# Lweihan/LDiffusion

Measured on AMD Instinct MI355X. Metric: patches/sec (512x512, 5 denoise steps), higher is better.
Workload: dtype f16 (fp32 accumulate)

## Files before the change

ldiffusion_amd/csrc/common.h:

```cpp
#pragma once
#include <hip/hip_runtime.h>
#include <stdint.h>
#include <stdio.h>
#include <string>
#include <vector>

typedef _Float16 f16;
typedef _Float16 f16x2 __attribute__((ext_vector_type(2)));
typedef _Float16 f16x4 __attribute__((ext_vector_type(4)));
typedef _Float16 f16x8 __attribute__((ext_vector_type(8)));
typedef float f32x4 __attribute__((ext_vector_type(4)));
typedef short s16x4 __attribute__((ext_vector_type(4)));

#include "../../include/ldiff.h"
void ldiff_set_error(const char* fmt, ...);

struct LdiffError {
  int code;
};
#define LDIFF_CHECK(cond, code, ...)     \
  do {                                   \
    if (!(cond)) {                       \
      ldiff_set_error(__VA_ARGS__);      \
      throw LdiffError{code};            \
// ... 56 lines not shown
  int silu_out = 0, cond_force = 0;
  int lrelu_in = 0, tconv = 0;
  int seg_conv = 0;
  int relu_out = 0, cls_force = 0;
  int* nonfinite = nullptr;
  int act_out = 0;
  int plan_B = 0, plan_M = 0;
};
inline ConvParams nominal_launch(const ConvParams& p) {
  ConvParams q = p;
  if (p.plan_B > 0) { q.B = p.plan_B; q.M = p.plan_M; }
  return q;
}
constexpr int LO8_SHIFT = 15;
void launch_lo8_weights(const f16* w, void* wd, int* scale_out, int Nrows, int taps, int Cin, hipStream_t s);
enum class ConvKernel { COND , TCONV , SEGCONV , CLSCONV , C3_NARROW, C3_NARROW_FOLD, C3_DATAFLOW, C3_PINGPONG, C3_HALO, GEMM_DF, GEMM_DMA, IGEMM, NONE  };
enum class ConvWeights { PLAIN, FRAG, FRAG_PAR, FRAG_SC, GEMM_FRAG };
struct ConvAsk {
  int splitk = 0;
  bool stats = false;
  bool fold_gn = false;
};
struct ConvPlan {
  ConvKernel kernel = ConvKernel::NONE;
  ConvWeights weights = ConvWeights::PLAIN;
  bool parity = false;
  bool fold_gn = false;
  int bm = 0, bn = 0;
};
ConvPlan plan_conv(ConvParams& p, const ConvAsk& ask);
size_t parity_weights_bytes(const ConvParams& p);
void pack_parity_weights(const ConvParams& p, f16* dst, hipStream_t s);
size_t packed_weights_bytes(ConvWeights layout, const ConvParams& p);
void pack_weights(ConvWeights layout, const ConvParams& p, const f16* sc_w, f16* dst, hipStream_t s);
void pack_shortcut_bias(const ConvParams& p, const float* sc_bias, float* dst, hipStream_t s);
bool conv_lo8_enabled();
void launch_igemm(const ConvParams& p, const ConvPlan& pl, hipStream_t s);
bool cond_conv_selected(const ConvParams& p);
void launch_cond_conv(const ConvParams& p, hipStream_t s);
void launch_tconv2x2(const ConvParams& p, hipStream_t s);
bool segconv_selected(const ConvParams& p);
int segconv_stats_blocks(const ConvParams& p);
void launch_segconv(const ConvParams& p, hipStream_t s);
void launch_in_finalize(const float* part, int R, const f16* x_or_null, int ldx, int B, int HW, int C, float eps, const float* gamma, const float* beta, float* scale, float* shift,
                        int ld_ss, int ss_off, int ident , hipStream_t s, int* nonfinite);
void launch_nhwc_f32_to_nchw(const float* x, void* y, int B, int C, int H, int W, int ldx, int out_f16, hipStream_t s);
bool cls_conv_selected(const ConvParams& p);
void launch_cls_conv(const ConvParams& p, hipStream_t s);
void launch_maxpool3x3s2(const f16* x, f16* y, int B, int H, int W, int C, hipStream_t s);
void launch_crop_resize_norm(const uint8_t* rgb, int H, int W, const int* boxes, int n, const uint8_t* lut, int S, const double* mean3, const double* std3, f16* out, hipStream_t s);
void launch_cls_head(const f16* x, int B, int HW, int A, int ldx, const float* w, const float* bias, int C, float* logits, int* labels_or_null, hipStream_t s);
void launch_scale_f16(const f16* x, f16* y, float a, long long n, hipStream_t s);
bool conv3x3_eligible(const ConvParams& p);
void launch_splitk_reduce(const ConvParams& p, hipStream_t s);
void launch_make_parity_weights(const f16* w, f16* w_par, int Nrows, int Cin, hipStream_t s);
void launch_conv3x3(const ConvParams& p, int bm, int bn, hipStream_t s);
bool conv3x3n_selected(const ConvParams& p);
bool conv3x3nt_selected(const ConvParams& p);
void launch_conv3x3n(const ConvParams& p, bool fold, hipStream_t s);
bool conv3x3p_selected(const ConvParams& p);
bool conv3x3d_selected(const ConvParams& p);
int conv3x3d_stats_blocks(const ConvParams& p);
size_t conv3x3d_frag_bytes(const ConvParams& p);
void launch_pack_frag_weights(const f16* w, f16* wf, int N, int Cin, hipStream_t s);
void launch_pack_frag_weights_par(const f16* wpar, f16* wf, int N, int Nrows, int Cin, hipStream_t s);
void launch_pack_frag_weights_sc(const f16* wsc, f16* wf, int N, int Cin, int Cs, int ld_wsc, hipStream_t s);
void launch_add_vectors(const float* a, const float* b, float* out, int n, hipStream_t s);
void launch_conv3x3d(const ConvParams& p, hipStream_t s);
int conv3x3p_stats_blocks(const ConvParams& p);
void launch_conv3x3p(const ConvParams& p, hipStream_t s);
bool lngemm_eligible(int C, int N, int ldx, int x_lo, int ldy, bool geglu);
void launch_lngemm_tile_weights(const f16* w, f16* wt, int N, int C, hipStream_t s);
void launch_lngemm(const f16* x, int ldx, int x_lo, int M, int C, const float* gamma, const float* beta, float eps, const f16* w_tiled, int N,
                   const float* bias, bool geglu, f16* y, int ldy, hipStream_t s, int qcols = 0, float qscale = 1.0f,
                   int plan_M = 0);
bool gemm_dma_eligible(const ConvParams& p);
bool gemm_df_selected(const ConvParams& p);
size_t gemm_df_frag_bytes(const ConvParams& p);
void launch_pack_gemm_frag(const f16* w, f16* wf, int Nrows, int K, hipStream_t s);
void launch_gemm_df(const ConvParams& p, hipStream_t s);
void launch_gemm_dma(const ConvParams& p, int bm, int bn, hipStream_t s);

struct AttnParams {
  const f16* q; int ldq;
  const f16* k; int ldk;
  const f16* v; int ldv;
  f16* o; int ldo;
  int B, heads, Lq, Lk, d;
  long long q_bstride, kv_bstride, o_bstride;
  float scale;
  int prescaled = 0;
  float rescale_log2 = 0.0f;
  int xcd_order = 0;
  int plan_B = 0;
};
void launch_attention(const AttnParams& p, hipStream_t s);
bool attention_prescale_supported(int d);

void launch_text_embed(const int* ids, const float* tok, const float* pos, f16* y, int M, int L, int H, int vocab, hipStream_t s);
bool text_attention_supported(int d, int L);
void launch_text_attention(const f16* qkv, int ld, int hidden, f16* o, int ldo, int o_lo , int B, int heads, int L, int d, float scale,
                           hipStream_t s);
void launch_text_ln(const f16* x_split, int M, int C, const float* gamma, const float* beta, float eps, void* out, int out_f16, f16* y_split, int* nonfinite, hipStream_t s);
void launch_f32_to_f16(const float* x, f16* y, long long n, hipStream_t s);

struct SrcView { const f16* p; int C, ld, lo; };
// ... 285 lines not shown
```

ldiffusion_amd/csrc/conv_route.hip:

```cpp
#include "common.h"

namespace {

long long tiles(const ConvParams& p, int bm, int bn) { return (long long)((p.M + bm - 1) / bm) * ((p.N + bn - 1) / bn); }
bool n_small(const ConvParams& p) { return p.N <= 64 || (p.N % 128 != 0 && p.N % 128 <= 64 && p.N < 512); }
int splits(long long t, int nk) { int S = (int)(512 / t); S = S > nk / 16 ? nk / 16 : S; return S > 8 ? 8 : S; }

int splitk_by_model(long long tiles, int steps, int min_steps, double partial_bytes, int s_old, int s_cap = 16) {
  auto T = [&](int S) {
    const double wgs = (double)tiles * S, per = (steps + S - 1) / S;
    return 4.0 + per * 0.95 * (wgs > 330.0 ? wgs / 330.0 : 1.0) + (S > 1 ? 4.0 + 2.0 * S * partial_bytes / 3.0e6 : 0.0);
  };
  if (s_old < 1) s_old = 1;
  int best = s_old;
  double tb = T(s_old);
  for (int S = s_old + 1; S <= s_cap && steps / S >= min_steps; ++S)
    if (T(S) < tb) { tb = T(S); best = S; }
  return tb <= 0.85 * T(s_old) ? best : s_old;
}

void c3_tile(const ConvParams& p, ConvPlan& pl) {
  pl.bm = (p.w_par ? p.Win : p.Wout) >= 16 ? 128 : 64;
  pl.bn = (p.N % 128 != 0 && p.N % 160 == 0) ? 160 : (p.N <= 32 ? 32 : (p.N <= 64 ? 64 : 128));
}
// ... 72 lines not shown
  LDIFF_CHECK(!q.act_out || !(q.relu_out || q.cls_force > 0 || q.silu_out || q.cond_force > 0 || q.tconv || q.lrelu_in || q.seg_conv > 0), LDIFF_ERR_INVALID,
              "conv: act_out cannot be combined with relu_out / cls_conv = 1 / silu_out / cond_conv = 1 / tconv / lrelu_in / seg_conv = 1 (only the LDS-DMA GEMM has that epilogue)");
  if (ask.splitk < 2 && cond_conv_selected(q)) {
    pl.kernel = ConvKernel::COND;
    p.splitk = 0;
    p.stats_R = 0;
    return pl;
  }
  LDIFF_CHECK(!q.lrelu_in || (q.gn_scale && q.gn_shift && !q.silu_in && (q.lrelu_in & ~3) == 0), LDIFF_ERR_INVALID, "conv: lrelu_in = %d needs gn_scale / gn_shift, silu_in = 0 and bits 0..1 only", q.lrelu_in);
  if (q.tconv) {
    LDIFF_CHECK(q.tconv == 1 && q.ks == 2 && q.stride == 2 && !q.ups && !q.x2 && q.C2 == 0 && q.C1 % 8 == 0 && q.Hout == 2 * q.Hin && q.Wout == 2 * q.Win && q.N == q.Nrows && q.N % 16 == 0 &&
                    q.K == q.C1 && !q.res && !q.temb && !q.out_f32 && !q.y_lo && !q.geglu && !q.silu_in && !q.silu_out && !q.out_shift && !q.xs && !q.lo8_slab0 && ask.splitk < 2 && !ask.stats &&
                    q.ldy >= q.N && q.ldy % 4 == 0 && (q.ld1 == 0 || (q.ld1 >= q.C1 && q.ld1 % 8 == 0)) && (long long)q.B * q.Hin * q.Win == q.M / 4 && q.M % 4 == 0,
                LDIFF_ERR_INVALID, "conv: tconv takes kernel = stride = 2, one source with C1 %% 8 == 0, N == Nrows, N %% 16 == 0, Hout = 2 Hin, a plain fp16 output and bias only (C1=%d N=%d Nrows=%d ks=%d stride=%d)",
                q.C1, q.N, q.Nrows, q.ks, q.stride);
    pl.kernel = ConvKernel::TCONV;
    p.splitk = 0;
    p.stats_R = 0;
    return pl;
  }
  if (ask.splitk < 2 && segconv_selected(q)) {
    pl.kernel = ConvKernel::SEGCONV;
    p.splitk = 0;
    p.stats_R = ask.stats ? segconv_stats_blocks(q) : 0;
    return pl;
  }
  if (ask.splitk < 2 && !ask.stats && cls_conv_selected(q)) {
    pl.kernel = ConvKernel::CLSCONV;
    p.splitk = 0;
    p.stats_R = 0;
    return pl;
  }
  LDIFF_CHECK(!q.relu_out && q.ks != 7, LDIFF_ERR_INVALID, "conv: a ReLU epilogue (relu_out) and 7x7 taps exist only in the classifier's conv family, which does not take this launch (Cin=%d N=%d ks=%d stride=%d pad=%d cls_conv=%d)",
              q.C1 + q.C2, q.N, q.ks, q.stride, q.pad_t, q.cls_force);
  LDIFF_CHECK(!q.silu_out, LDIFF_ERR_INVALID, "conv: a SiLU epilogue (silu_out) exists only in the conditioning-embedding kernel, which does not take this launch (Cin=%d N=%d ks=%d stride=%d)",
              q.C1 + q.C2, q.N, q.ks, q.stride);
  if (q.act_out) {
    LDIFF_CHECK((q.act_out == 1 || q.act_out == 2) && !q.geglu && !q.res && !q.out_f32 && !q.out_shift && !q.gn_scale && !q.temb && !ask.stats && ask.splitk < 2 && q.w_bstride == 0 &&
                    !q.xs && !q.lo8_slab0 && p.df_force <= 0 && gemm_dma_eligible(q),
                LDIFF_ERR_INVALID, "conv: act_out = %d (1 quick_gelu | 2 gelu) exists only in the LDS-DMA GEMM: a linear layer (ks = 1, K %% 64 == 0) with bias and an fp16 output (plain or split), no residual / "
                "fp32 output / GEGLU / statistics / range shift / split-K / gemm_df (C1=%d C2=%d N=%d ks=%d stride=%d)", q.act_out, q.C1, q.C2, q.N, q.ks, q.stride);
    pl.kernel = ConvKernel::GEMM_DMA;
    gemm_dma_tile(q, 1, pl);
    p.splitk = 0;
    p.stats_R = 0;
    return pl;
  }
  if (ask.fold_gn && q.gn_scale && !q.silu_in && !q.lrelu_in && q.ks == 1 && !q.x2 && !q.out_f32 && !q.geglu) {
    ConvParams f = q;
    f.gn_scale = nullptr; f.gn_shift = nullptr;
    f.w_bstride = (long long)q.Nrows * q.K; f.bias_bstride = q.Nrows;
    if (gemm_dma_eligible(f)) { q = f; pl.fold_gn = true; }
  }
  const bool c3 = conv3x3_eligible(q) && !(q.lrelu_in && q.ups), gemm = !c3 && !q.lrelu_in && gemm_dma_eligible(q);
  pl.parity = q.ups && c3;
  if (pl.parity) q.w_par = reinterpret_cast<const f16*>(placeholder);
  if (ask.splitk >= 2) {
    LDIFF_CHECK(ask.splitk <= (c3 ? (q.C1 + q.C2) / 64 : (q.K + 63) / 64), LDIFF_ERR_INVALID, "conv: more splits than K steps (%d)", ask.splitk);
    q.splitk = ask.splitk;
  } else if (ask.splitk == 0 && !q.out_f32) {
    q.splitk = c3 ? conv3x3_splitk_plan(q) : gemm ? gemm_dma_splitk_plan(q) : igemm_splitk_plan(q);
  }
  if (q.splitk < 2) q.splitk = 0;
  const int hw = q.Hout * q.Wout;
  const bool rows32 = q.splitk > 1 || !c3;
  q.stats = nullptr; q.stats_R = 0;
  if (ask.stats && !q.out_f32 && hw > 0 && (!rows32 || hw % 32 == 0)) {
    q.stats = placeholder;
    q.stats_R = rows32 ? hw / 32 : 0;
  }
  if (c3) {
    const bool par = pl.parity;
    const int Ht = par ? q.Hin : q.Hout, Wt = par ? q.Win : q.Wout;
    if (q.lrelu_in) {
      pl.kernel = ConvKernel::C3_HALO;
      c3_tile(q, pl);
    } else if (q.lo8_slab0) pl.kernel = q.splitk <= 1 && conv3x3p_selected(q) ? ConvKernel::C3_PINGPONG : ConvKernel::NONE;
    else if (conv3x3n_selected(q)) pl.kernel = conv3x3nt_selected(q) ? ConvKernel::C3_NARROW_FOLD : ConvKernel::C3_NARROW;
    else if (conv3x3d_selected(q)) pl.kernel = ConvKernel::C3_DATAFLOW;
    else if (conv3x3p_selected(q)) pl.kernel = ConvKernel::C3_PINGPONG;
    else {
      pl.kernel = ConvKernel::C3_HALO;
      c3_tile(q, pl);
    }
    if (q.stats && !rows32) {
      if (q.lo8_slab0 || pl.kernel == ConvKernel::C3_PINGPONG) q.stats_R = conv3x3p_stats_blocks(q);
      else if (pl.kernel == ConvKernel::C3_DATAFLOW) q.stats_R = conv3x3d_stats_blocks(q);
      else {
        const int TW = pl.bm / 8;
        q.stats_R = ((Ht + 7) / 8) * ((Wt + TW - 1) / TW) * (TW == 16 ? 1 : 2) * (par ? 4 : 1);
      }
    }
  } else if (gemm) {
    if (gemm_df_selected(q)) pl.kernel = ConvKernel::GEMM_DF;
    else {
      pl.kernel = ConvKernel::GEMM_DMA;
      gemm_dma_tile(q, q.splitk > 1 ? q.splitk : 1, pl);
    }
  } else {
    pl.kernel = ConvKernel::IGEMM;
    igemm_tile(q, q.splitk > 1 ? q.splitk : 1, pl);
  }
  if (pl.kernel == ConvKernel::C3_DATAFLOW) pl.weights = q.xs ? ConvWeights::FRAG_SC : pl.parity ? ConvWeights::FRAG_PAR : ConvWeights::FRAG;
  else if (pl.kernel == ConvKernel::GEMM_DF) pl.weights = ConvWeights::GEMM_FRAG;

  p.splitk = q.splitk;
  p.stats_R = q.stats_R;
  if (pl.fold_gn) {
    p.gn_scale = nullptr; p.gn_shift = nullptr;
    p.w_bstride = q.w_bstride; p.bias_bstride = q.bias_bstride;
  }
  return pl;
}

size_t parity_weights_bytes(const ConvParams& p) { return (size_t)4 * p.Nrows * 4 * (p.C1 + p.C2) * sizeof(f16); }
void pack_parity_weights(const ConvParams& p, f16* dst, hipStream_t s) { launch_make_parity_weights(p.w, dst, p.Nrows, p.C1 + p.C2, s); }
size_t packed_weights_bytes(ConvWeights layout, const ConvParams& p) {
  return layout == ConvWeights::PLAIN ? 0 : layout == ConvWeights::GEMM_FRAG ? gemm_df_frag_bytes(p) : conv3x3d_frag_bytes(p);
}
void pack_weights(ConvWeights layout, const ConvParams& p, const f16* sc_w, f16* dst, hipStream_t s) {
  switch (layout) {
    case ConvWeights::PLAIN: break;
    case ConvWeights::FRAG_PAR: launch_pack_frag_weights_par(p.w_par, dst, p.N, p.Nrows, p.C1, s); break;
    case ConvWeights::FRAG:
    case ConvWeights::FRAG_SC:
      launch_pack_frag_weights(p.w, dst, p.N, p.C1, s);
      if (layout == ConvWeights::FRAG_SC) launch_pack_frag_weights_sc(sc_w, dst, p.N, p.C1, p.Cs, p.Cs, s);
// ... 6 lines not shown
```

ldiffusion_amd/csrc/kernels_conv3x3.hip:

```cpp
#include "common.h"

namespace {

__device__ __forceinline__ int swz8(int row, int chunk) { return chunk ^ ((row >> 1) & 7); }

typedef __attribute__((address_space(1))) const void gptr_t;
typedef __attribute__((address_space(3))) void lptr_t;

template <int TH, int TW, int BN, bool GN, bool LR = false>
__global__ __launch_bounds__(256, 2) void conv3x3_kernel(const ConvParams p) {
  constexpr int BM = TH * TW, HWD = TW + 2, HP = (TH + 2) * (TW + 2);
  constexpr int MT = BM / 32, NT = BN / 32;
  constexpr int A_IT = (HP * 8 + 255) / 256, W_IT = BN * 8 / 256;
  static_assert(BN % 32 == 0 && (BN * 8) % 256 == 0, "BN must be a multiple of 32");
  extern __shared__ __attribute__((aligned(16))) unsigned char smem_raw[];
  uint4* sA = reinterpret_cast<uint4*>(smem_raw);
  uint4* sW = sA + 2 * HP * 8;

  const int tid = threadIdx.x, lane = tid & 63;
  const int wave = __builtin_amdgcn_readfirstlane(tid >> 6);
  const int wave_m = wave >> 1, wave_n = wave & 1;
  const int g = lane >> 4, l15 = lane & 15;
  const int Cin = p.C1 + p.C2;
  const bool par = p.w_par != nullptr;
// ... 212 lines not shown
      if (p.res) { v += up4(rr[m][a]); if (p.res_lo) v += up4(rl[m][a]); }
      if (p.out_f32) {
        *reinterpret_cast<f32x4*>(reinterpret_cast<float*>(p.y) + mrow[m] * p.ldy + n) = v;
      } else {
        const f16x4 o = cvt4(v);
        *reinterpret_cast<f16x4*>(reinterpret_cast<f16*>(p.y) + mrow[m] * p.ldy + n) = o;
        if (p.y_lo) *reinterpret_cast<f16x4*>(reinterpret_cast<f16*>(p.y) + mrow[m] * p.ldy + p.y_lo + n) = cvt4(v - up4(o));
        if (p.stats) acc[a][m] = p.y_lo ? split_stat4(v) : up4(o);
      }
    }
  }
  if (p.stats) {
    bool ok[MT];
#pragma unroll
    for (int m = 0; m < MT; ++m) ok[m] = mrow[m] >= 0;
    const long long R = p.stats_R, rblk = (((long long)q_par * tiles_y + ty) * tiles_x + tx) * 2 + wave_m;
    wave_stats_store<MT, NT>(acc, ok, 0, MT, p.stats + ((long long)b * p.N * R + rblk) * 2, R, p.N, ncol, l15);
  }
}

template <int I, int N, class F>
__device__ __forceinline__ void static_for(F&& f) {
  if constexpr (I < N) { f(std::integral_constant<int, I>{}); static_for<I + 1, N>(f); }
}
template <int OFF>
__device__ __forceinline__ void lds_read128(f16x8& d, unsigned addr) {
  asm volatile("ds_read_b128 %0, %1 offset:%2" : "=v"(d) : "v"(addr), "n"(OFF) : "memory");
}
template <int CNT>
__device__ __forceinline__ void lds_wait(f16x8& a) { asm volatile("s_waitcnt lgkmcnt(%1)" : "+v"(a) : "n"(CNT)); }
template <int CNT>
__device__ __forceinline__ void lds_wait(f16x8& a, f16x8& b, f16x8& c, f16x8& d, f16x8& e) {
  asm volatile("s_waitcnt lgkmcnt(%5)" : "+v"(a), "+v"(b), "+v"(c), "+v"(d), "+v"(e) : "n"(CNT));
}

__device__ __forceinline__ int swzx(int hx) { return (0xcb5888 >> (3 * (hx >> 1))) & 7; }

#ifdef C3W_STAMPS
__device__ unsigned long long c3w_dbg[32];
__device__ __forceinline__ unsigned long long w_stamp() {
  __builtin_amdgcn_sched_barrier(0);
  unsigned long long t = __builtin_amdgcn_s_memtime();
  asm volatile("s_waitcnt lgkmcnt(0)" ::: "memory");
  __builtin_amdgcn_sched_barrier(0);
  return t;
}
#define WSTAMP(v) const unsigned long long v = w_stamp()
#define WACC(i, expr) wdbg[i] += (expr)
#else
#define WSTAMP(v)
#define WACC(i, expr)
#endif

template <int BN, bool GN, bool LR = false>
__global__ __launch_bounds__(256, BN > 128 ? 1 : 2) void conv3x3w_kernel(const ConvParams p) {
  constexpr int TH = 8, TW = 16, BM = 128, HWD = 18, HP = 180, MT = 4, NT = BN / 32, A_IT = 6, NP = BN / 32;
  constexpr int ROWB = HWD * 128;
#ifdef C3W_RING2
  constexpr bool R3 = false;
#else
  constexpr bool R3 = BN == 160;
#endif
  constexpr int NSLOT = R3 ? 3 : 2;
  constexpr unsigned W_OFF = 2 * HP * 128, W_BYTES = BN * 128;
  constexpr unsigned DUMP = W_OFF + NSLOT * W_BYTES;
  constexpr int NF = NT + MT;
  extern __shared__ __attribute__((aligned(16))) unsigned char smem_raw[];

  const int tid = threadIdx.x, lane = tid & 63;
  const int wave = __builtin_amdgcn_readfirstlane(tid >> 6);
  const int wave_m = wave >> 1, wave_n = wave & 1;
  const int g = lane >> 4, l15 = lane & 15;
  const int Cin = p.C1 + p.C2;
  const bool par = p.w_par != nullptr;
  const int Ht = par ? p.Hin : p.Hout, Wt = par ? p.Win : p.Wout;
  const int tiles_x = (Wt + TW - 1) / TW, tiles_y = (Ht + TH - 1) / TH;
  const int ntn = (p.N + BN - 1) / BN;
  int nwg = gridDim.x, id = blockIdx.x;
  int q8 = nwg >> 3, r8 = nwg & 7, xcd = id & 7, idx = id >> 3;
  int sw = (xcd < r8 ? xcd * (q8 + 1) : r8 * (q8 + 1) + (xcd - r8) * q8) + idx;
  auto fdiv = [](int n, unsigned m) { return m ? (int)__umulhi((unsigned)n, m) : n; };
  int tm, tile_n;
  if (p.img_fast) { tile_n = fdiv(sw, p.div_tm); tm = sw - tile_n * p.tiles_m; }
  else { tm = fdiv(sw, p.div_ntn); tile_n = sw - tm * ntn; }
  const int q_par = par ? tm & 3 : 0, py = q_par >> 1, px = q_par & 1;
  tm = par ? tm >> 2 : tm;
  const int tq = fdiv(tm, p.div_tx);
  const int tx = tm - tq * tiles_x;
  const int b = fdiv(tq, p.div_ty);
  const int ty = tq - b * tiles_y;
  const int n0 = tile_n * BN, oy0 = ty * TH, ox0 = tx * TW;
  const int sh = par ? 0 : p.ups;
  const int He = p.Hin << sh, We = p.Win << sh;
  const unsigned lds0 = (unsigned)(size_t)(lptr_t*)smem_raw;
#ifdef C3W_STAMPS
  unsigned long long wdbg[32] = {0};
  WSTAMP(w_t0);
#endif

  const int kc = tid & 7;
  unsigned a_pix[A_IT], a_msk[A_IT], a_lds[A_IT];
#pragma unroll
  for (int i = 0; i < A_IT; ++i) {
    const int hp = (tid >> 3) + i * 32;
    const int hy = hp / HWD, hx = hp - hy * HWD;
    const int iy = oy0 + hy - 1, ix = ox0 + hx - 1;
    const bool inb = hp < HP && iy >= 0 && iy < He && ix >= 0 && ix < We;
    a_pix[i] = inb ? (unsigned)(((b * p.Hin + (iy >> sh)) * p.Win) + (ix >> sh)) : 0u;
    a_msk[i] = inb ? 0xffffffffu : 0u;
    a_lds[i] = hp < HP ? (unsigned)(hp * 128 + ((kc ^ swzx(hx)) << 4)) : DUMP + (unsigned)((tid - 160) * 16);
  }
  uint4 ra[A_IT];
  float4 gs0, gs1, gt0, gt1;
  float lslope = 1.0f;
  auto load_halo = [&](int c) {
    const int cb = c * 64;
    const f16* src; int cs, Cs;
    if (cb < p.C1) { src = p.x; cs = cb; Cs = p.ld1 ? p.ld1 : p.C1; } else { src = p.x2; cs = cb - p.C1; Cs = p.ld2 ? p.ld2 : p.C2; }
    if (LR) lslope = ((cb < p.C1 ? p.lrelu_in : p.lrelu_in >> 1) & 1) ? 0.01f : 1.0f;
    src += cs + kc * 8;
#pragma unroll
    for (int i = 0; i < A_IT; ++i) ra[i] = *reinterpret_cast<const uint4*>(src + (size_t)a_pix[i] * (unsigned)Cs);
    if (GN) {
      const float* sc = p.gn_scale + (long long)b * Cin + cb + kc * 8;
      const float* st = p.gn_shift + (long long)b * Cin + cb + kc * 8;
      gs0 = *reinterpret_cast<const float4*>(sc); gs1 = *reinterpret_cast<const float4*>(sc + 4);
      gt0 = *reinterpret_cast<const float4*>(st); gt1 = *reinterpret_cast<const float4*>(st + 4);
    }
  };
  const int nslab_all = Cin >> 6, S = p.splitk > 1 ? p.splitk : 1, ksplit = blockIdx.y;
  int c_begin = 0, nslab = nslab_all;
  if (S > 1) { c_begin = ksplit * nslab_all / S; nslab = (ksplit + 1) * nslab_all / S; }
  load_halo(c_begin);
  __builtin_amdgcn_sched_barrier(0);
  const bool silu = p.silu_in != 0;
  auto xform_store = [&](auto ic, unsigned bufoff) {
    constexpr int i = decltype(ic)::value;
    uint4 v = ra[i];
    if constexpr (LR) {
      v.x = in_lrelu_pair(ra[i].x, gs0.x, gt0.x, gs0.y, gt0.y, lslope); v.y = in_lrelu_pair(ra[i].y, gs0.z, gt0.z, gs0.w, gt0.w, lslope);
      v.z = in_lrelu_pair(ra[i].z, gs1.x, gt1.x, gs1.y, gt1.y, lslope); v.w = in_lrelu_pair(ra[i].w, gs1.z, gt1.z, gs1.w, gt1.w, lslope);
    } else if (GN) {
      if (silu) {
        v.x = gn_pair<true>(ra[i].x, gs0.x, gt0.x, gs0.y, gt0.y); v.y = gn_pair<true>(ra[i].y, gs0.z, gt0.z, gs0.w, gt0.w);
        v.z = gn_pair<true>(ra[i].z, gs1.x, gt1.x, gs1.y, gt1.y); v.w = gn_pair<true>(ra[i].w, gs1.z, gt1.z, gs1.w, gt1.w);
      } else {
        v.x = gn_pair<false>(ra[i].x, gs0.x, gt0.x, gs0.y, gt0.y); v.y = gn_pair<false>(ra[i].y, gs0.z, gt0.z, gs0.w, gt0.w);
        v.z = gn_pair<false>(ra[i].z, gs1.x, gt1.x, gs1.y, gt1.y); v.w = gn_pair<false>(ra[i].w, gs1.z, gt1.z, gs1.w, gt1.w);
      }
    }
    v.x &= a_msk[i]; v.y &= a_msk[i]; v.z &= a_msk[i]; v.w &= a_msk[i];
    *reinterpret_cast<uint4*>(smem_raw + bufoff + a_lds[i]) = v;
  };

  const long long Kw = (long long)(par ? 4 : 9) * Cin;
  const f16* wsrc = par ? p.w_par + (long long)q_par * p.Nrows * Kw : p.w;
  const __amdgpu_buffer_rsrc_t wrsrc = __builtin_amdgcn_make_buffer_rsrc((void*)wsrc, 0, (int)((long long)p.Nrows * Kw * 2), 0x00020000);
  int w_voff[NP];
#pragma unroll
  for (int i = 0; i < NP; ++i) {
    const int r = wave * (BN / 4) + i * 8 + (lane >> 3), pos = lane & 7;
    int n = n0 + r;
    n = n < p.Nrows ? n : p.Nrows - 1;
    w_voff[i] = (int)(((long long)n * Kw + swz8(r, pos) * 8) * 2) - (i & 3) * 1024;
  }
  auto issue_w_piece = [&](auto ic, int soff, unsigned slot) {
    constexpr int i = decltype(ic)::value;
    unsigned char* dst = smem_raw + W_OFF + slot * W_BYTES + wave * (BN * 32);
#if defined(__HIP_DEVICE_COMPILE__)
    __builtin_amdgcn_raw_ptr_buffer_load_lds(wrsrc, (lptr_t*)(dst + (i >> 2) * 4096), 16, w_voff[i], soff, (i & 3) * 1024, 0);
#endif
  };
  auto issue_w = [&](int soff, unsigned slot) {
    unsigned char* dst = smem_raw + W_OFF + slot * W_BYTES + wave * (BN * 32);
    static_for<0, NP>([&](auto ic) {
      constexpr int i = decltype(ic)::value;
#if defined(__HIP_DEVICE_COMPILE__)
      __builtin_amdgcn_raw_ptr_buffer_load_lds(wrsrc, (lptr_t*)(dst + (i >> 2) * 4096), 16, w_voff[i], soff, (i & 3) * 1024, 0);
#endif
    });
  };

  f32x4 acc[NT][MT];
#pragma unroll
  for (int a = 0; a < NT; ++a)
#pragma unroll
    for (int m = 0; m < MT; ++m) acc[a][m] = (f32x4){0.f, 0.f, 0.f, 0.f};

  unsigned xb[3];
#pragma unroll
  for (int j = 0; j < 3; ++j) {
    const int hx = l15 + (par ? px + (j & 1) : j);
    xb[j] = lds0 + (unsigned)(((wave_m * 4 + (par ? py : 0)) * HWD + hx) * 128 + ((g ^ swzx(hx)) << 4));
  }
  const int wrow = wave_n * (BN / 2) + l15;
  const unsigned w_lane = lds0 + W_OFF + (unsigned)(wrow * 128 + ((g ^ ((wrow >> 1) & 7)) << 4));

  issue_w(c_begin * 128, 0);
  if (R3 && !par) issue_w((Cin + c_begin * 64) * 2, 1);
  static_for<0, A_IT>([&](auto ic) { xform_store(ic, 0u); });
  __syncthreads();

  auto xform_pair = [&](auto ic, auto dc, auto siluc) -> unsigned {
    constexpr int i = decltype(ic)::value, d = decltype(dc)::value;
    if constexpr (LR) return in_lrelu_pair(dword4<d>(ra[i]), comp8<2 * d>(gs0, gs1), comp8<2 * d>(gt0, gt1), comp8<2 * d + 1>(gs0, gs1), comp8<2 * d + 1>(gt0, gt1), lslope);
    else return gn_pair<decltype(siluc)::value>(dword4<d>(ra[i]), comp8<2 * d>(gs0, gs1), comp8<2 * d>(gt0, gt1), comp8<2 * d + 1>(gs0, gs1), comp8<2 * d + 1>(gt0, gt1));
  };
  auto mask_store = [&](auto ic, uint4 v, unsigned bufoff) {
    constexpr int i = decltype(ic)::value;
    v.x &= a_msk[i]; v.y &= a_msk[i]; v.z &= a_msk[i]; v.w &= a_msk[i];
    *reinterpret_cast<uint4*>(smem_raw + bufoff + a_lds[i]) = v;
  };

  auto run = [&](auto parc, auto siluc) {
    constexpr bool PAR = decltype(parc)::value;
    constexpr int NTAPS = PAR ? 4 : 9, CPT = PAR ? 2 : 1;
    unsigned sp = 0;
    auto slab = [&](int c, auto stagec) {
      constexpr bool STAGE = decltype(stagec)::value, stage = STAGE;
      const unsigned hbuf = (unsigned)((c - c_begin) & 1) * (HP * 128);
      unsigned xc[3], xc1[3], wc[2], wc1[2];
#pragma unroll
      for (int j = 0; j < 3; ++j) { xc[j] = xb[j] + hbuf; xc1[j] = xc[j] ^ 64u; }
      wc[0] = w_lane + sp * W_BYTES; wc[1] = w_lane + (sp ^ 1u) * W_BYTES;
      wc1[0] = wc[0] ^ 64u; wc1[1] = wc[1] ^ 64u;
      constexpr bool RING3 = R3 && !PAR;
      static_for<0, NTAPS>([&](auto tc) {
        constexpr int T = decltype(tc)::value;
        constexpr int kyi = PAR ? (T >> 1) : T / 3, kxi = PAR ? (T & 1) : T % 3;
        constexpr bool LAST = T == NTAPS - 1;
        constexpr int C0 = T >= 1 ? (T - 1) * CPT : A_IT, C1 = T >= 1 ? (T * CPT < A_IT ? T * CPT : A_IT) : A_IT;
        constexpr int NE = GN && STAGE && C0 < C1 ? (C1 - C0) * 4 : 0, EPG = (NE + NT - 1) / NT;
        unsigned pk[NE > 0 ? NE : 1];
        f16x8 wf[2][NT], xf[2][MT];
        WSTAMP(s0);
        const unsigned wcur = RING3 ? w_lane + (unsigned)(T % 3) * W_BYTES : wc[T & 1], wcur1 = wcur ^ 64u;
        constexpr int T2 = T + 2;
        constexpr bool DMA_NOW = RING3 && (T2 < NTAPS || STAGE);
        const int soff2 = T2 < NTAPS ? (T2 * Cin + c * 64) * 2 : ((T2 - NTAPS) * Cin + (c + 1) * 64) * 2;
        static_for<0, MT>([&](auto mc) { constexpr int m = decltype(mc)::value; lds_read128<(m + kyi) * ROWB>(xf[0][m], xc[kxi]); });
        static_for<0, NT>([&](auto ac) { constexpr int a = decltype(ac)::value; lds_read128<a * 2048>(wf[0][a], wcur); });
        __builtin_amdgcn_sched_barrier(0);
        if constexpr (!RING3) {
          if (!LAST) issue_w(((T + 1) * Cin + c * 64) * 2, sp ^ (unsigned)((T + 1) & 1));
          else if (stage) issue_w((c + 1) * 128, sp ^ (unsigned)(NTAPS & 1));
        }
        if (T == 0 && stage) load_halo(c + 1);
        __builtin_amdgcn_sched_barrier(0);
        WSTAMP(s1);
        static_for<0, 2 * NT>([&](auto ic) {
          constexpr int kk = decltype(ic)::value / NT, a = decltype(ic)::value % NT;
          constexpr int WI = NT > 1 ? 1 : 0;
          constexpr int pending = kk == 1 ? NT - 1 - a : (NT - 1 - a) + (a >= 1 ? MT : 0) + (a > WI ? NT : 0);
          if constexpr (a == 0) lds_wait<pending>(xf[kk][0], xf[kk][1], xf[kk][2], xf[kk][3], wf[kk][0]);
          else lds_wait<pending>(wf[kk][a]);
#pragma unroll
          for (int m = 0; m < MT; ++m)
            acc[a][m] = __builtin_amdgcn_mfma_f32_16x16x32_f16(wf[kk][a], xf[kk][m], acc[a][m], 0, 0, 0);
          if constexpr (kk == 0 && a == 0) static_for<0, MT>([&](auto mc) { constexpr int m = decltype(mc)::value; lds_read128<(m + kyi) * ROWB>(xf[1][m], xc1[kxi]); });
          if constexpr (kk == 0 && a == WI) static_for<0, NT>([&](auto bc) { constexpr int b2 = decltype(bc)::value; lds_read128<b2 * 2048>(wf[1][b2], wcur1); });
          if constexpr (DMA_NOW && kk == 0 && a < NP) issue_w_piece(std::integral_constant<int, a>{}, soff2, (unsigned)(T2 % 3));
          static_for<(kk == 1 ? a * EPG : NE), (kk == 1 ? ((a + 1) * EPG < NE ? (a + 1) * EPG : NE) : NE)>([&](auto ec) {
            constexpr int e = decltype(ec)::value;
            pk[e] = xform_pair(std::integral_constant<int, C0 + e / 4>{}, std::integral_constant<int, e % 4>{}, siluc);
          });
          __builtin_amdgcn_sched_barrier(0);
        });
        if constexpr (STAGE) static_for<C0, C1>([&](auto ic) {
          constexpr int i = decltype(ic)::value;
          uint4 v = ra[i];
          if constexpr (GN) v = make_uint4(pk[(i - C0) * 4], pk[(i - C0) * 4 + 1], pk[(i - C0) * 4 + 2], pk[(i - C0) * 4 + 3]);
          mask_store(ic, v, (unsigned)(HP * 128) - hbuf);
        });
        WSTAMP(s2);
        if constexpr (RING3) {
          if constexpr (DMA_NOW) asm volatile("s_waitcnt vmcnt(%0) lgkmcnt(0)" ::"n"(NP) : "memory");
          else asm volatile("s_waitcnt vmcnt(0) lgkmcnt(0)" ::: "memory");
          __builtin_amdgcn_s_barrier();
        } else __syncthreads();
        WSTAMP(s3);
        WACC(1, s1 - s0); WACC(2, s2 - s1); WACC(3, s3 - s2); WACC(4, 1); WACC(8 + T, s2 - s1); WACC(20 + T, s1 - s0);
      });
      sp ^= (unsigned)(NTAPS & 1);
    };
    for (int c = c_begin; c + 1 < nslab; ++c) slab(c, std::true_type{});
    slab(nslab - 1, std::false_type{});
  };
  if (GN && silu) { if (par) run(std::true_type{}, std::true_type{}); else run(std::false_type{}, std::true_type{}); }
  else { if (par) run(std::true_type{}, std::false_type{}); else run(std::false_type{}, std::false_type{}); }
#ifdef C3W_STAMPS
  { WSTAMP(w_t1); wdbg[0] = w_t1 - w_t0; }
  if (blockIdx.x == 0 && blockIdx.y == 0 && threadIdx.x == 0) for (int i = 0; i < 32; ++i) c3w_dbg[i] = wdbg[i];
#endif

  if (S > 1) {
    const int ncol_s = n0 + wave_n * (BN / 2) + g * 4;
#pragma unroll
    for (int m = 0; m < MT; ++m) {
      const int ml = wave_m * (BM / 2) + m * 16 + l15;
      const int ty_ = oy0 + ml / TW, tx_ = ox0 + ml % TW;
      const int oy = par ? 2 * ty_ + py : ty_, ox = par ? 2 * tx_ + px : tx_;
      if (ty_ >= Ht || tx_ >= Wt) continue;
      const long long mrow_s = ((long long)b * p.Hout + oy) * p.Wout + ox;
#pragma unroll
      for (int a = 0; a < NT; ++a) {
        const int n = ncol_s + a * 16;
        if (n < p.N) *reinterpret_cast<f32x4*>(p.splitk_ws + ((long long)ksplit * p.M + mrow_s) * p.N + n) = acc[a][m];
      }
    }
    return;
  }
  const int ncol = n0 + wave_n * (BN / 2) + g * 4;
  const float osc = shift_scale(p.out_shift);
  f32x4 bt[NT];
#pragma unroll
  for (int a = 0; a < NT; ++a) {
    const int n = ncol + a * 16;
    float4 bb = make_float4(0.f, 0.f, 0.f, 0.f), tt = make_float4(0.f, 0.f, 0.f, 0.f);
    if (n < p.N) {
      if (p.bias) bb = *reinterpret_cast<const float4*>(p.bias + n);
      if (p.temb) tt = *reinterpret_cast<const float4*>(p.temb + (long long)b * p.ld_temb + n);
    }
    bt[a] = (f32x4){bb.x + tt.x, bb.y + tt.y, bb.z + tt.z, bb.w + tt.w};
  }
  long long mrow[MT];
#pragma unroll
  for (int m = 0; m < MT; ++m) {
    const int ml = wave_m * (BM / 2) + m * 16 + l15;
    const int ty_ = oy0 + ml / TW, tx_ = ox0 + ml % TW;
    const int oy = par ? 2 * ty_ + py : ty_, ox = par ? 2 * tx_ + px : tx_;
    mrow[m] = (ty_ < Ht && tx_ < Wt) ? ((long long)b * p.Hout + oy) * p.Wout + ox : -1;
  }
  f16x4 rr[MT][NT], rl[MT][NT];
  if (p.res) {
#pragma unroll
    for (int m = 0; m < MT; ++m)
#pragma unroll
      for (int a = 0; a < NT; ++a) {
        rr[m][a] = (f16x4){(f16)0.f, (f16)0.f, (f16)0.f, (f16)0.f};
        rl[m][a] = rr[m][a];
        if (mrow[m] >= 0 && ncol + a * 16 < p.N) {
// ... 186 lines not shown
    const int rblk = (int)(m0 - b * hw) >> 5;
    *reinterpret_cast<float2*>(p.stats + ((b * p.N + blockIdx.y * 64 + tid) * (long long)p.stats_R + rblk) * 2) = make_float2(a, q);
  }
}

void launch_splitk_reduce_impl(const ConvParams& p, hipStream_t s) {
  LDIFF_CHECK(p.splitk >= 2 && p.splitk <= SPLITK_MAX && p.splitk_ws && (p.N & 3) == 0, LDIFF_ERR_INVALID, "split-K reduce: %d splits (at most %d)", p.splitk, SPLITK_MAX);
  if (p.stats) {
    const int hw = p.Hout * p.Wout;
    LDIFF_CHECK(!p.out_f32 && hw % 32 == 0 && p.stats_R == hw / 32 && p.M % 32 == 0, LDIFF_ERR_INVALID, "split-K reduce: fused statistics need 32 | H W and R = H W / 32 (R = %d)", p.stats_R);
    const dim3 grid((unsigned)(p.M / 32), (unsigned)((p.N + 63) / 64));
    if (p.splitk <= 8) hipLaunchKernelGGL(splitk_reduce_stats_kernel<8>, grid, dim3(256), 0, s, p);
    else hipLaunchKernelGGL(splitk_reduce_stats_kernel<16>, grid, dim3(256), 0, s, p);
  } else {
    const long long n = (long long)p.M * (p.N >> 2);
    const dim3 grid((unsigned)((n + 255) / 256));
    if (p.splitk <= 8) hipLaunchKernelGGL(splitk_reduce_kernel<8>, grid, dim3(256), 0, s, p);
    else hipLaunchKernelGGL(splitk_reduce_kernel<16>, grid, dim3(256), 0, s, p);
  }
  HIP_CHECK(hipGetLastError());
}

static bool conv3x3_img_fast(const ConvParams& p, int tiles_per_image, int ntn, int bn) {
  static const int mode = [] { const char* e = getenv("LDIFF_CONV3X3_IMGFAST"); return e ? atoi(e) : -1; }();
  if (mode == 0 || ntn <= 1 || (p.plan_B > 0 ? p.plan_B : p.B) <= 1) return false;
  if (mode > 0) return tiles_per_image <= mode;
  (void)bn;
  return tiles_per_image <= 2;
}

template <int TH, int TW, int BN, bool GN, bool LR = false>
void launch_c3(const ConvParams& p, hipStream_t s) {
  constexpr int HP = (TH + 2) * (TW + 2);
  const size_t smem = (size_t)(2 * HP * 8 + 2 * BN * 8) * 16;
  auto kern = conv3x3_kernel<TH, TW, BN, GN, LR>;
  ensure_dyn_smem(reinterpret_cast<const void*>(kern), (int)smem);
  const bool par = p.w_par != nullptr;
  const int Ht = par ? p.Hin : p.Hout, Wt = par ? p.Win : p.Wout;
  const int tiles = p.B * ((Ht + TH - 1) / TH) * ((Wt + TW - 1) / TW);
  const int ntn = (p.N + BN - 1) / BN;
  static const std::string pname = std::string(LR ? "conv3x3_lrelu<" : "conv3x3<") + std::to_string(TH) + "x" + std::to_string(TW) + "," + std::to_string(BN) + (GN && !LR ? ",gn>" : ">");
  const double bytes = (double)p.B * p.Hin * p.Win * (p.C1 + p.C2) * 2.0 + (double)p.N * p.K * 2.0 + (double)p.M * p.N * (p.out_f32 ? 4.0 : (p.y_lo ? 4.0 : 2.0)) +
                       (p.res ? (double)p.M * p.N * (p.res_lo ? 4.0 : 2.0) : 0.0);
  ProfScope prof(pname.c_str(), 2.0 * p.M * (double)p.N * p.K * (par ? 16.0 / 36.0 : 1.0), bytes, s);
  const int S = p.splitk > 1 ? p.splitk : 1;
  ConvParams q = p;
  const int npar = par ? 4 : 1;
  q.tiles_m = tiles * npar; q.img_fast = conv3x3_img_fast(p, tiles / p.B, ntn, BN) ? 1 : 0;
  hipLaunchKernelGGL(kern, dim3(tiles * ntn * npar, S, 1), dim3(256), smem, s, q);
  HIP_CHECK(hipGetLastError());
  if (S > 1) launch_splitk_reduce_impl(p, s);
}

template <int BN, bool GN, bool LR = false>
void launch_c3w(const ConvParams& p, hipStream_t s) {
  constexpr int TH = 8, TW = 16, HP = 180;
  const size_t smem = (size_t)2 * HP * 128 + (BN == 160 ? 3 : 2) * BN * 128 + 1536;
  auto kern = conv3x3w_kernel<BN, GN, LR>;
  ensure_dyn_smem(reinterpret_cast<const void*>(kern), (int)smem);
  const bool par = p.w_par != nullptr;
  const int Ht = par ? p.Hin : p.Hout, Wt = par ? p.Win : p.Wout;
  const int tiles = p.B * ((Ht + TH - 1) / TH) * ((Wt + TW - 1) / TW);
  const int ntn = (p.N + BN - 1) / BN;
  static const std::string pname = std::string(LR ? "conv3x3_lrelu<8x16," : "conv3x3<8x16,") + std::to_string(BN) + (GN && !LR ? ",gn>" : ">");
  const double bytes = (double)p.B * p.Hin * p.Win * (p.C1 + p.C2) * 2.0 + (double)p.N * p.K * 2.0 + (double)p.M * p.N * (p.out_f32 ? 4.0 : (p.y_lo ? 4.0 : 2.0)) +
                       (p.res ? (double)p.M * p.N * (p.res_lo ? 4.0 : 2.0) : 0.0);
  ProfScope prof(pname.c_str(), 2.0 * p.M * (double)p.N * p.K * (par ? 16.0 / 36.0 : 1.0), bytes, s);
  const int S = p.splitk > 1 ? p.splitk : 1;
  const int tiles_x = (Wt + TW - 1) / TW, tiles_y = (Ht + TH - 1) / TH;
  LDIFF_CHECK((long long)tiles * (par ? 4 : 1) * ntn * std::max(std::max(ntn, tiles * (par ? 4 : 1)), std::max(tiles_x, tiles_y)) < (1LL << 32), LDIFF_ERR_INVALID, "conv3x3: %d tiles x %d channel tiles exceed the tile decode's range", tiles, ntn);
  ConvParams q = p;
  auto recip = [](int d) { return d == 1 ? 0u : (unsigned)((1ULL << 32) / (unsigned)d + 1ULL); };
  q.div_ntn = recip(ntn); q.div_tx = recip(tiles_x); q.div_ty = recip(tiles_y);
  const int npar = par ? 4 : 1;
  q.tiles_m = tiles * npar; q.div_tm = recip(tiles * npar); q.img_fast = conv3x3_img_fast(p, tiles / p.B, ntn, BN) ? 1 : 0;
  hipLaunchKernelGGL(kern, dim3(tiles * ntn * npar, S, 1), dim3(256), smem, s, q);
  HIP_CHECK(hipGetLastError());
  if (S > 1) launch_splitk_reduce_impl(p, s);
}
template <int BN>
void launch_c3w_gn(const ConvParams& p, hipStream_t s) {
  if (p.lrelu_in) launch_c3w<BN, true, true>(p, s);
  else if (p.gn_scale) launch_c3w<BN, true>(p, s); else launch_c3w<BN, false>(p, s);
}

template <int TH, int TW, int BN>
void launch_c3_gn(const ConvParams& p, hipStream_t s) {
  if (p.lrelu_in) launch_c3<TH, TW, BN, true, true>(p, s);
  else if (p.gn_scale) launch_c3<TH, TW, BN, true>(p, s); else launch_c3<TH, TW, BN, false>(p, s);
}

}

__global__ void make_parity_weights_kernel(const f16* __restrict__ w, f16* __restrict__ wp, int Nrows, int Cin) {
  const long long i = (long long)blockIdx.x * blockDim.x + threadIdx.x;
  const long long total = 4LL * Nrows * 4 * Cin;
  if (i >= total) return;
  const int c = (int)(i % Cin);
  const int t = (int)((i / Cin) % 4);
  const int n = (int)((i / (4LL * Cin)) % Nrows);
  const int q = (int)(i / (4LL * Cin * Nrows));
  const int py = q >> 1, px = q & 1, ty = t >> 1, tx = t & 1;
  const int ky0 = py == 0 ? (ty == 0 ? 0 : 1) : (ty == 0 ? 0 : 2), ky1 = py == 0 ? (ty == 0 ? 0 : 2) : (ty == 0 ? 1 : 2);
  const int kx0 = px == 0 ? (tx == 0 ? 0 : 1) : (tx == 0 ? 0 : 2), kx1 = px == 0 ? (tx == 0 ? 0 : 2) : (tx == 0 ? 1 : 2);
  float acc = 0.f;
  for (int ky = ky0; ky <= ky1; ++ky)
    for (int kx = kx0; kx <= kx1; ++kx) acc += (float)w[((long long)n * 9 + ky * 3 + kx) * Cin + c];
  wp[i] = (f16)acc;
}
void launch_make_parity_weights(const f16* w, f16* w_par, int Nrows, int Cin, hipStream_t s) {
  const long long total = 4LL * Nrows * 4 * Cin;
  hipLaunchKernelGGL(make_parity_weights_kernel, dim3((unsigned)((total + 255) / 256)), dim3(256), 0, s, w, w_par, Nrows, Cin);
  HIP_CHECK(hipGetLastError());
}

bool conv3x3_eligible(const ConvParams& p) {
  const int Cin = p.C1 + p.C2;
  return p.ks == 3 && p.stride == 1 && p.pad_t == 1 && p.pad_l == 1 && Cin % 64 == 0 && p.C1 % 64 == 0 && (long long)p.Nrows * 9 * Cin * 2 < (1LL << 32) &&
         p.Hout == (p.Hin << p.ups) && p.Wout == (p.Win << p.ups);
}

void launch_splitk_reduce(const ConvParams& p, hipStream_t s) { launch_splitk_reduce_impl(p, s); }

void launch_conv3x3(const ConvParams& p, int bm, int bn, hipStream_t s) {
  if (bm == 128) {
    if (bn == 160) launch_c3w_gn<160>(p, s);
    else if (bn == 64) launch_c3w_gn<64>(p, s);
    else if (bn == 32) launch_c3w_gn<32>(p, s);
    else launch_c3w_gn<128>(p, s);
  } else {
    if (bn == 160) launch_c3_gn<8, 8, 160>(p, s);
    else if (bn == 64) launch_c3_gn<8, 8, 64>(p, s);
    else if (bn == 32) launch_c3_gn<8, 8, 32>(p, s);
    else launch_c3_gn<8, 8, 128>(p, s);
  }
}

#ifdef C3W_STAMPS
extern "C" int ldiff_debug_c3w_stamps(unsigned long long* out) {
  return (int)hipMemcpyFromSymbol(out, HIP_SYMBOL(c3w_dbg), sizeof(unsigned long long) * 32);
}
#endif
```

Baseline: 51.66.

## Route stride-2 3x3 convolutions through the 8x16 implicit-GEMM kernel via parity planes

Adds a stride-2 variant of the wide 3x3 conv kernel. The input halo is split into four parity planes (even/odd rows and columns) that are loaded one after another, and the taps are reordered so each plane's taps run together from LDS. Qualifying downsampling convs (no GN prologue, large enough spatial size) are routed to this kernel instead of the generic implicit GEMM. The aim is better data reuse and MFMA pipelining for downsampling layers. In exchange the halo is loaded four times per channel slab and double-buffering across slabs is reduced, which could expose load latency.

After: 51.98, median of 6. Within noise of the previous version (+0.6%).

```diff
diff --git a/ldiffusion_amd/csrc/common.h b/ldiffusion_amd/csrc/common.h
--- a/ldiffusion_amd/csrc/common.h
+++ b/ldiffusion_amd/csrc/common.h
@@ -132,6 +132,7 @@
 void launch_cls_head(const f16* x, int B, int HW, int A, int ldx, const float* w, const float* bias, int C, float* logits, int* labels_or_null, hipStream_t s);
 void launch_scale_f16(const f16* x, f16* y, float a, long long n, hipStream_t s);
 bool conv3x3_eligible(const ConvParams& p);
+bool conv3x3s2_selected(const ConvParams& p);
 void launch_splitk_reduce(const ConvParams& p, hipStream_t s);
 void launch_make_parity_weights(const f16* w, f16* w_par, int Nrows, int Cin, hipStream_t s);
 void launch_conv3x3(const ConvParams& p, int bm, int bn, hipStream_t s);
diff --git a/ldiffusion_amd/csrc/conv_route.hip b/ldiffusion_amd/csrc/conv_route.hip
--- a/ldiffusion_amd/csrc/conv_route.hip
+++ b/ldiffusion_amd/csrc/conv_route.hip
@@ -148,7 +148,8 @@
     f.w_bstride = (long long)q.Nrows * q.K; f.bias_bstride = q.Nrows;
     if (gemm_dma_eligible(f)) { q = f; pl.fold_gn = true; }
   }
-  const bool c3 = conv3x3_eligible(q) && !(q.lrelu_in && q.ups), gemm = !c3 && !q.lrelu_in && gemm_dma_eligible(q);
+  const bool c3s2 = conv3x3s2_selected(q);
+  const bool c3 = c3s2 || (conv3x3_eligible(q) && !(q.lrelu_in && q.ups)), gemm = !c3 && !q.lrelu_in && gemm_dma_eligible(q);
   pl.parity = q.ups && c3;
   if (pl.parity) q.w_par = reinterpret_cast<const f16*>(placeholder);
   if (ask.splitk >= 2) {
@@ -168,7 +169,7 @@
   if (c3) {
     const bool par = pl.parity;
     const int Ht = par ? q.Hin : q.Hout, Wt = par ? q.Win : q.Wout;
-    if (q.lrelu_in) {
+    if (c3s2 || q.lrelu_in) {
       pl.kernel = ConvKernel::C3_HALO;
       c3_tile(q, pl);
     } else if (q.lo8_slab0) pl.kernel = q.splitk <= 1 && conv3x3p_selected(q) ? ConvKernel::C3_PINGPONG : ConvKernel::NONE;
diff --git a/ldiffusion_amd/csrc/kernels_conv3x3.hip b/ldiffusion_amd/csrc/kernels_conv3x3.hip
--- a/ldiffusion_amd/csrc/kernels_conv3x3.hip
+++ b/ldiffusion_amd/csrc/kernels_conv3x3.hip
@@ -288,8 +288,16 @@
 #define WACC(i, expr)
 #endif
 
-template <int BN, bool GN, bool LR = false>
+constexpr int c3s2_tap[9] = {0, 2, 6, 8, 1, 7, 3, 5, 4};
+constexpr int c3s2_sy[9] = {0, 0, 1, 1, 0, 1, 0, 0, 0};
+constexpr int c3s2_sx[9] = {0, 1, 0, 1, 0, 0, 0, 1, 0};
+constexpr int c3s2_pl[9] = {0, 0, 0, 0, 1, 1, 2, 2, 3};
+constexpr bool c3s2_first(int T) { return T == 0 || c3s2_pl[T] != c3s2_pl[T - 1]; }
+constexpr bool c3s2_last(int T) { return T == 8 || c3s2_pl[T] != c3s2_pl[T + 1]; }
+
+template <int BN, bool GN, bool LR = false, bool S2 = false>
 __global__ __launch_bounds__(256, BN > 128 ? 1 : 2) void conv3x3w_kernel(const ConvParams p) {
+  static_assert(!S2 || (!GN && !LR), "the stride-2 form has no prologue");
   constexpr int TH = 8, TW = 16, BM = 128, HWD = 18, HP = 180, MT = 4, NT = BN / 32, A_IT = 6, NP = BN / 32;
   constexpr int ROWB = HWD * 128;
 #ifdef C3W_RING2
@@ -308,7 +316,7 @@
   const int wave_m = wave >> 1, wave_n = wave & 1;
   const int g = lane >> 4, l15 = lane & 15;
   const int Cin = p.C1 + p.C2;
-  const bool par = p.w_par != nullptr;
+  const bool par = !S2 && p.w_par != nullptr;
   const int Ht = par ? p.Hin : p.Hout, Wt = par ? p.Win : p.Wout;
   const int tiles_x = (Wt + TW - 1) / TW, tiles_y = (Ht + TH - 1) / TH;
   const int ntn = (p.N + BN - 1) / BN;
@@ -336,12 +344,17 @@
 
   const int kc = tid & 7;
   unsigned a_pix[A_IT], a_msk[A_IT], a_lds[A_IT];
+  int s_iy[S2 ? A_IT : 1], s_ix[S2 ? A_IT : 1];
 #pragma unroll
   for (int i = 0; i < A_IT; ++i) {
     const int hp = (tid >> 3) + i * 32;
     const int hy = hp / HWD, hx = hp - hy * HWD;
+    if constexpr (S2) {
+      s_iy[i] = hp < HP && hy <= TH && hx <= TW ? 2 * (oy0 + hy) - p.pad_t : -4;
+      s_ix[i] = 2 * (ox0 + hx) - p.pad_l;
+    }
     const int iy = oy0 + hy - 1, ix = ox0 + hx - 1;
-    const bool inb = hp < HP && iy >= 0 && iy < He && ix >= 0 && ix < We;
+    const bool inb = !S2 && hp < HP && iy >= 0 && iy < He && ix >= 0 && ix < We;
     a_pix[i] = inb ? (unsigned)(((b * p.Hin + (iy >> sh)) * p.Win) + (ix >> sh)) : 0u;
     a_msk[i] = inb ? 0xffffffffu : 0u;
     a_lds[i] = hp < HP ? (unsigned)(hp * 128 + ((kc ^ swzx(hx)) << 4)) : DUMP + (unsigned)((tid - 160) * 16);
@@ -349,12 +362,21 @@
   uint4 ra[A_IT];
   float4 gs0, gs1, gt0, gt1;
   float lslope = 1.0f;
-  auto load_halo = [&](int c) {
+  auto load_halo = [&](int c, int pl = 0) {
     const int cb = c * 64;
     const f16* src; int cs, Cs;
     if (cb < p.C1) { src = p.x; cs = cb; Cs = p.ld1 ? p.ld1 : p.C1; } else { src = p.x2; cs = cb - p.C1; Cs = p.ld2 ? p.ld2 : p.C2; }
     if (LR) lslope = ((cb < p.C1 ? p.lrelu_in : p.lrelu_in >> 1) & 1) ? 0.01f : 1.0f;
     src += cs + kc * 8;
+    if constexpr (S2) {
+#pragma unroll
+      for (int i = 0; i < A_IT; ++i) {
+        const int iy = s_iy[i] + (pl >> 1), ix = s_ix[i] + (pl & 1);
+        const bool inb = (unsigned)iy < (unsigned)p.Hin && (unsigned)ix < (unsigned)p.Win;
+        a_pix[i] = inb ? (unsigned)((b * p.Hin + iy) * p.Win + ix) : 0u;
+        a_msk[i] = inb ? 0xffffffffu : 0u;
+      }
+    }
 #pragma unroll
     for (int i = 0; i < A_IT; ++i) ra[i] = *reinterpret_cast<const uint4*>(src + (size_t)a_pix[i] * (unsigned)Cs);
     if (GN) {
@@ -433,7 +455,7 @@
   const unsigned w_lane = lds0 + W_OFF + (unsigned)(wrow * 128 + ((g ^ ((wrow >> 1) & 7)) << 4));
 
   issue_w(c_begin * 128, 0);
-  if (R3 && !par) issue_w((Cin + c_begin * 64) * 2, 1);
+  if (R3 && !par) issue_w(((S2 ? c3s2_tap[1] : 1) * Cin + c_begin * 64) * 2, 1);
   static_for<0, A_IT>([&](auto ic) { xform_store(ic, 0u); });
   __syncthreads();
 
@@ -454,7 +476,7 @@
     unsigned sp = 0;
     auto slab = [&](int c, auto stagec) {
       constexpr bool STAGE = decltype(stagec)::value, stage = STAGE;
-      const unsigned hbuf = (unsigned)((c - c_begin) & 1) * (HP * 128);
+      const unsigned hbuf = S2 ? 0u : (unsigned)((c - c_begin) & 1) * (HP * 128);
       unsigned xc[3], xc1[3], wc[2], wc1[2];
 #pragma unroll
       for (int j = 0; j < 3; ++j) { xc[j] = xb[j] + hbuf; xc1[j] = xc[j] ^ 64u; }
@@ -463,9 +485,14 @@
       constexpr bool RING3 = R3 && !PAR;
       static_for<0, NTAPS>([&](auto tc) {
         constexpr int T = decltype(tc)::value;
-        constexpr int kyi = PAR ? (T >> 1) : T / 3, kxi = PAR ? (T & 1) : T % 3;
+        constexpr int kyi = S2 ? c3s2_sy[T % 9] : PAR ? (T >> 1) : T / 3, kxi = S2 ? c3s2_sx[T % 9] : PAR ? (T & 1) : T % 3;
         constexpr bool LAST = T == NTAPS - 1;
-        constexpr int C0 = T >= 1 ? (T - 1) * CPT : A_IT, C1 = T >= 1 ? (T * CPT < A_IT ? T * CPT : A_IT) : A_IT;
+        constexpr int PL = S2 ? c3s2_pl[T % 9] : 0;
+        constexpr unsigned XOFF = S2 ? (unsigned)(PL & 1) * (HP * 128) : 0u;
+        constexpr bool S2_LOAD = S2 && c3s2_first(T % 9) && (PL < 3 || STAGE);
+        constexpr bool S2_STORE = S2 && c3s2_last(T % 9) && (PL < 3 || STAGE);
+        constexpr auto wtap = [](int t) { return S2 ? c3s2_tap[t % 9] : t; };
+        constexpr int C0 = S2 ? (S2_STORE ? 0 : A_IT) : T >= 1 ? (T - 1) * CPT : A_IT, C1 = S2 ? A_IT : T >= 1 ? (T * CPT < A_IT ? T * CPT : A_IT) : A_IT;
         constexpr int NE = GN && STAGE && C0 < C1 ? (C1 - C0) * 4 : 0, EPG = (NE + NT - 1) / NT;
         unsigned pk[NE > 0 ? NE : 1];
         f16x8 wf[2][NT], xf[2][MT];
@@ -473,15 +500,16 @@
         const unsigned wcur = RING3 ? w_lane + (unsigned)(T % 3) * W_BYTES : wc[T & 1], wcur1 = wcur ^ 64u;
         constexpr int T2 = T + 2;
         constexpr bool DMA_NOW = RING3 && (T2 < NTAPS || STAGE);
-        const int soff2 = T2 < NTAPS ? (T2 * Cin + c * 64) * 2 : ((T2 - NTAPS) * Cin + (c + 1) * 64) * 2;
-        static_for<0, MT>([&](auto mc) { constexpr int m = decltype(mc)::value; lds_read128<(m + kyi) * ROWB>(xf[0][m], xc[kxi]); });
+        const int soff2 = T2 < NTAPS ? (wtap(T2) * Cin + c * 64) * 2 : (wtap(T2 - NTAPS) * Cin + (c + 1) * 64) * 2;
+        static_for<0, MT>([&](auto mc) { constexpr int m = decltype(mc)::value; lds_read128<(m + kyi) * ROWB + XOFF>(xf[0][m], xc[kxi]); });
         static_for<0, NT>([&](auto ac) { constexpr int a = decltype(ac)::value; lds_read128<a * 2048>(wf[0][a], wcur); });
         __builtin_amdgcn_sched_barrier(0);
         if constexpr (!RING3) {
-          if (!LAST) issue_w(((T + 1) * Cin + c * 64) * 2, sp ^ (unsigned)((T + 1) & 1));
+          if (!LAST) issue_w((wtap(T + 1) * Cin + c * 64) * 2, sp ^ (unsigned)((T + 1) & 1));
           else if (stage) issue_w((c + 1) * 128, sp ^ (unsigned)(NTAPS & 1));
         }
-        if (T == 0 && stage) load_halo(c + 1);
+        if constexpr (S2) { if constexpr (S2_LOAD) load_halo(PL < 3 ? c : c + 1, (PL + 1) & 3); }
+        else if (T == 0 && stage) load_halo(c + 1);
         __builtin_amdgcn_sched_barrier(0);
         WSTAMP(s1);
         static_for<0, 2 * NT>([&](auto ic) {
@@ -493,7 +521,7 @@
 #pragma unroll
           for (int m = 0; m < MT; ++m)
             acc[a][m] = __builtin_amdgcn_mfma_f32_16x16x32_f16(wf[kk][a], xf[kk][m], acc[a][m], 0, 0, 0);
-          if constexpr (kk == 0 && a == 0) static_for<0, MT>([&](auto mc) { constexpr int m = decltype(mc)::value; lds_read128<(m + kyi) * ROWB>(xf[1][m], xc1[kxi]); });
+          if constexpr (kk == 0 && a == 0) static_for<0, MT>([&](auto mc) { constexpr int m = decltype(mc)::value; lds_read128<(m + kyi) * ROWB + XOFF>(xf[1][m], xc1[kxi]); });
           if constexpr (kk == 0 && a == WI) static_for<0, NT>([&](auto bc) { constexpr int b2 = decltype(bc)::value; lds_read128<b2 * 2048>(wf[1][b2], wcur1); });
           if constexpr (DMA_NOW && kk == 0 && a < NP) issue_w_piece(std::integral_constant<int, a>{}, soff2, (unsigned)(T2 % 3));
           static_for<(kk == 1 ? a * EPG : NE), (kk == 1 ? ((a + 1) * EPG < NE ? (a + 1) * EPG : NE) : NE)>([&](auto ec) {
@@ -502,11 +530,11 @@
           });
           __builtin_amdgcn_sched_barrier(0);
         });
-        if constexpr (STAGE) static_for<C0, C1>([&](auto ic) {
+        if constexpr (STAGE || S2) static_for<C0, C1>([&](auto ic) {
           constexpr int i = decltype(ic)::value;
           uint4 v = ra[i];
           if constexpr (GN) v = make_uint4(pk[(i - C0) * 4], pk[(i - C0) * 4 + 1], pk[(i - C0) * 4 + 2], pk[(i - C0) * 4 + 3]);
-          mask_store(ic, v, (unsigned)(HP * 128) - hbuf);
+          mask_store(ic, v, S2 ? (unsigned)((PL + 1) & 1) * (HP * 128) : (unsigned)(HP * 128) - hbuf);
         });
         WSTAMP(s2);
         if constexpr (RING3) {
@@ -522,7 +550,8 @@
     for (int c = c_begin; c + 1 < nslab; ++c) slab(c, std::true_type{});
     slab(nslab - 1, std::false_type{});
   };
-  if (GN && silu) { if (par) run(std::true_type{}, std::true_type{}); else run(std::false_type{}, std::true_type{}); }
+  if constexpr (S2) run(std::false_type{}, std::false_type{});
+  else if (GN && silu) { if (par) run(std::true_type{}, std::true_type{}); else run(std::false_type{}, std::true_type{}); }
   else { if (par) run(std::true_type{}, std::false_type{}); else run(std::false_type{}, std::false_type{}); }
 #ifdef C3W_STAMPS
   { WSTAMP(w_t1); wdbg[0] = w_t1 - w_t0; }
@@ -815,11 +844,11 @@
   if (S > 1) launch_splitk_reduce_impl(p, s);
 }
 
-template <int BN, bool GN, bool LR = false>
+template <int BN, bool GN, bool LR = false, bool S2 = false>
 void launch_c3w(const ConvParams& p, hipStream_t s) {
   constexpr int TH = 8, TW = 16, HP = 180;
   const size_t smem = (size_t)2 * HP * 128 + (BN == 160 ? 3 : 2) * BN * 128 + 1536;
-  auto kern = conv3x3w_kernel<BN, GN, LR>;
+  auto kern = conv3x3w_kernel<BN, GN, LR, S2>;
   ensure_dyn_smem(reinterpret_cast<const void*>(kern), (int)smem);
   const bool par = p.w_par != nullptr;
   const int Ht = par ? p.Hin : p.Hout, Wt = par ? p.Win : p.Wout;
@@ -877,6 +906,15 @@
   HIP_CHECK(hipGetLastError());
 }
 
+bool conv3x3s2_selected(const ConvParams& p) {
+  const bool pad1 = p.pad_t == 1 && p.pad_l == 1 && p.Hout == (p.Hin - 1) / 2 + 1 && p.Wout == (p.Win - 1) / 2 + 1;
+  const bool pad0 = p.pad_t == 0 && p.pad_l == 0 && p.Hout == p.Hin / 2 && p.Wout == p.Win / 2;
+  const long long hw = (long long)p.Hout * p.Wout;
+  return p.ks == 3 && p.stride == 2 && !p.tconv && !p.x2 && p.C2 == 0 && p.C1 > 0 && p.C1 % 64 == 0 && (pad1 || pad0) && !p.gn_scale && !p.lrelu_in && !p.silu_in && !p.ups &&
+         !p.lo8_slab0 && !p.out_f32 && !p.geglu && p.w_bstride == 0 && !p.xs && p.Wout >= 16 && p.Hin >= 2 && (long long)p.Nrows * 9 * p.C1 * 2 < (1LL << 31) &&
+         (long long)p.B * p.Hin * p.Win < (1LL << 31) && (hw >= 1024 || (hw >= 256 && p.C1 >= 1024));
+}
+
 bool conv3x3_eligible(const ConvParams& p) {
   const int Cin = p.C1 + p.C2;
   return p.ks == 3 && p.stride == 1 && p.pad_t == 1 && p.pad_l == 1 && Cin % 64 == 0 && p.C1 % 64 == 0 && (long long)p.Nrows * 9 * Cin * 2 < (1LL << 32) &&
@@ -886,6 +924,15 @@
 void launch_splitk_reduce(const ConvParams& p, hipStream_t s) { launch_splitk_reduce_impl(p, s); }
 
 void launch_conv3x3(const ConvParams& p, int bm, int bn, hipStream_t s) {
+  if (p.stride == 2) {
+    LDIFF_CHECK(bm == 128 && conv3x3s2_selected(nominal_launch(p)), LDIFF_ERR_INVALID, "conv3x3: a stride-2 launch the 8 x 16 kernel does not take (C1=%d N=%d %dx%d -> %dx%d pad %d)", p.C1, p.N, p.Hin,
+                p.Win, p.Hout, p.Wout, p.pad_t);
+    if (bn == 160) launch_c3w<160, false, false, true>(p, s);
+    else if (bn == 64) launch_c3w<64, false, false, true>(p, s);
+    else if (bn == 32) launch_c3w<32, false, false, true>(p, s);
+    else launch_c3w<128, false, false, true>(p, s);
+    return;
+  }
   if (bm == 128) {
     if (bn == 160) launch_c3w_gn<160>(p, s);
     else if (bn == 64) launch_c3w_gn<64>(p, s);
```
